# yifanlu0227/HEAL

Hardware: AMD Instinct MI355X
Metric: scenes/sec (5-agent OPV2V-H, PointPillars+PyramidFusion) (higher is better)
Workload: dtype f32

## Files before the change

heal_amd/_capi.py:

```python
import ctypes
import os
import re

HERE = os.path.dirname(os.path.abspath(__file__))
LIB_PATH = os.environ.get("HEAL_AMD_LIB") or os.path.join(HERE, "lib", "libheal_amd.so")
HEADER = os.path.join(os.path.dirname(HERE), "include", "heal_amd.h")
HEADER_EXPERIMENTAL = os.path.join(os.path.dirname(HERE), "include", "heal_amd_experimental.h")

_lib = None

c_void_p, c_int, c_float, c_size_t = ctypes.c_void_p, ctypes.c_int, ctypes.c_float, ctypes.c_size_t

_SIGNATURES = {
    "heal_abi_version": (c_int, []),
    "heal_last_error": (ctypes.c_char_p, []),
    "heal_fill_bytes": (c_int, [c_void_p, c_int, c_size_t, c_void_p]),
    "heal_next_launch_events": (c_int, [c_void_p, c_void_p]),
    "heal_voxelize_workspace": (c_size_t, [c_int, c_int, c_int, ctypes.c_longlong]),
    "heal_voxelize": (c_int, [c_void_p, c_int, c_void_p, c_void_p, c_int, c_int, c_int,
                              c_void_p, c_void_p, c_void_p, c_void_p, c_void_p, c_void_p, c_void_p, c_size_t, c_int, c_void_p]),
    "heal_voxelize_batch_workspace": (c_size_t, [c_int, c_int, c_int, c_int, ctypes.c_longlong]),
    "heal_voxelize_batch": (c_int, [c_void_p, c_void_p, c_int, c_void_p, c_void_p, c_int, c_int, c_void_p, c_void_p,
                                    c_void_p, c_void_p, c_void_p, c_size_t, c_int, c_void_p]),
    "heal_mask_points": (c_int, [c_void_p, c_int, c_void_p, c_int, c_void_p, c_void_p]),
    "heal_pfn_scatter_workspace": (c_size_t, [c_int] * 5),
    "heal_pfn_scatter": (c_int, [c_void_p, c_void_p, c_void_p, c_int, c_void_p, c_int,
                                 c_void_p, c_void_p, c_void_p, c_int,
                                 c_float, c_float, c_float, c_float, c_float, c_float,
                                 c_int, c_int, c_int, c_void_p, c_void_p, c_void_p, c_size_t, c_void_p]),
    "heal_pfn_pillars": (c_int, [c_void_p, c_void_p, c_void_p, c_int, c_void_p, c_int, c_void_p, c_void_p, c_void_p, c_int,
                                 c_float, c_float, c_float, c_float, c_float, c_float, c_int, c_int, c_int, c_void_p, c_void_p,
                                 c_void_p]),
    "heal_pillar_canvas": (c_int, [c_void_p, c_void_p, c_int, c_int, c_int, c_int, c_void_p, c_void_p]),
    "heal_pillar_stem_block": (c_int, [c_void_p, c_void_p, c_int, c_int, c_int, c_int] + [c_void_p] * 4 + [c_int] + [c_void_p] * 3),
    "heal_bev_pool_backward": (c_int, [c_void_p] * 5 + [c_int] * 6 + [c_void_p] * 6),
    "heal_warp_fuse": (c_int, [c_void_p, c_void_p, c_int, c_int, c_int, c_int, c_void_p, c_void_p, c_int, c_void_p,
                               c_void_p, c_void_p]),
    "heal_warp_fuse_levels": (c_int, [c_int, c_void_p, c_void_p, c_int, c_void_p, c_void_p, c_void_p, c_void_p, c_void_p, c_int,
                                      c_void_p, c_void_p, c_void_p]),
    "heal_warp_att_fuse_levels": (c_int, [c_int, c_void_p, c_int, c_void_p, c_void_p, c_void_p, c_void_p, c_void_p, c_void_p, c_int,
                                          c_int, c_void_p, c_void_p]),
    "heal_disco_fuse": (c_int, [c_void_p, c_int, c_int, c_int, c_int, c_void_p, c_void_p, c_int] + [c_void_p] * 11),
    "heal_warp_fuse_backward": (c_int, [c_void_p, c_void_p, c_int, c_int, c_int, c_int, c_void_p, c_void_p, c_int, c_void_p,
                                        c_void_p, c_void_p, c_void_p, c_void_p]),
    "heal_warp_agent": (c_int, [c_void_p, c_void_p, c_int, c_int, c_int, c_void_p, c_void_p, c_int, c_void_p,
                                c_void_p, c_void_p, c_void_p]),
    "heal_warp_agents_pm": (c_int, [c_void_p, c_int, c_int, c_int, c_int, c_void_p, c_void_p, c_int, c_void_p, c_void_p]),
    "heal_fuse_warped": (c_int, [c_void_p, c_void_p, c_int, c_int, c_int, c_int, c_void_p, c_void_p]),
    "heal_fuse_warped_rows": (c_int, [c_void_p, c_void_p, c_void_p, c_int, c_int, c_int, c_int, c_void_p, c_void_p]),
    "heal_decode_nms_workspace": (c_size_t, [c_int, c_int]),
    "heal_decode_nms": (c_int, [c_void_p, c_void_p, c_void_p, c_void_p, c_int, c_int, c_int, c_int,
                                c_float, c_float, c_float, c_int, c_void_p, c_void_p,
                                c_void_p, c_void_p, c_void_p, c_int, c_void_p, c_size_t, c_void_p]),
    "heal_decode_nms_agents_workspace": (c_size_t, [c_int, c_int]),
# ... 283 lines not shown
```

heal_amd/csrc/warp_fuse.hip:

```cpp
#include <stdlib.h>
#include "common.h"
#include "warp_taps.h"
#include "../../include/heal_amd.h"

namespace heal {

constexpr int WF_TW = 32, WF_TH = 8;

struct WarpParams {
    const double* mdev;
    double m[WF_MAXA][6];
    int crop[WF_MAXA][4];
    int n_agents, C, H, W;
    int grid_f64;
};

__device__ __forceinline__ void load_affine(const WarpParams& p, int a, double (&m)[6]) {
#pragma unroll
    for (int k = 0; k < 6; ++k) m[k] = p.mdev ? p.mdev[a * 6 + k] : p.m[a][k];
}

__device__ __forceinline__ float score_at(const float* __restrict__ occ, int idx, int W, const int* crop) {
    if (crop[1] > crop[0]) {
        const int h = idx / W, w = idx - h * W;
// ... 107 lines not shown
                    }
                }
            }
        }
#pragma unroll
        for (int u = 0; u < U; ++u)
            if (c + u < p.C) out[(size_t)(c + u) * HW + pix] = acc[u];
    }
}

constexpr int WL_T = 16;
constexpr int WL_BMAX = 32;
constexpr int WL_CC = 8;
constexpr int WL_MAXL = 4;

struct WfLevel {
    const float* feats;
    const float* occ;
    float* out;
    int C, H, W;
    int tiles_x, cgroups, cpb;
    int block0;
    int crop[WF_MAXA][4];
};
struct WfLevels {
    WfLevel lv[WL_MAXL];
    int n_levels, n_agents, grid_f64, dbg;
    const double* mdev;
    double m[WF_MAXA][6];
};

template <int NA>
__global__ __launch_bounds__(256) void k_warp_fuse_lds(const WfLevels P) {
    __shared__ float s_box_f[WL_CC * WL_BMAX * (WL_BMAX + 1)];
    __shared__ int s_box[WF_MAXA][4];
    int lvl = 0;
#pragma unroll
    for (int i = 1; i < WL_MAXL; ++i)
        if (i < P.n_levels && (int)blockIdx.x >= P.lv[i].block0) lvl = i;
    const WfLevel& L = P.lv[lvl];
    const int lb = blockIdx.x - L.block0;
    const int cg = lb % L.cgroups, tile = lb / L.cgroups;
    const int tx0 = (tile % L.tiles_x) * WL_T, ty0 = (tile / L.tiles_x) * WL_T;
    const int tid = threadIdx.x;
    const int w = tx0 + (tid & (WL_T - 1)), h = ty0 + (tid >> 4);
// ... 23 lines not shown
        for (int k = 0; k < 4; ++k) wt[a][k] = 0.f;
        if (live) {
            float gx, gy;
            double m[6];
#pragma unroll
            for (int k = 0; k < 6; ++k) m[k] = P.mdev ? P.mdev[a * 6 + k] : P.m[a][k];
            if (P.grid_f64) {
                const double xs = s_base_d[0][tid & (WL_T - 1)], ys = s_base_d[1][tid >> 4];
                gx = (float)((m[0] * xs + m[1] * ys) + m[2]);
                gy = (float)((m[3] * xs + m[4] * ys) + m[5]);
            } else {
                const float xs = s_base_f[0][tid & (WL_T - 1)], ys = s_base_f[1][tid >> 4];
                gx = (float)(((float)m[0] * xs + (float)m[1] * ys) + (float)m[2]);
                gy = (float)(((float)m[3] * xs + (float)m[4] * ys) + (float)m[5]);
            }
            const Taps t = make_taps(gx, gy, L.H, L.W);
            prob[a] = sample_score(L.occ + (size_t)a * HW, t, L.W, L.crop[a]);
            const float ix = ((gx + 1.f) * (float)L.W - 1.f) / 2.f, iy = ((gy + 1.f) * (float)L.H - 1.f) / 2.f;
            tx[a] = (int)fminf(fmaxf(floorf(ix), -2.f), (float)L.W);
            ty[a] = (int)fminf(fmaxf(floorf(iy), -2.f), (float)L.H);
            okb[a] = t.ok;
#pragma unroll
            for (int k = 0; k < 4; ++k) wt[a][k] = ((t.ok >> k) & 1u) ? t.w[k] : 0.f;
        }
    }
    agent_softmax(prob, NA);
#pragma unroll
    for (int a = 0; a < NA; ++a) {
#pragma unroll
        for (int k = 0; k < 4; ++k) wt[a][k] *= prob[a];
        const bool any = (wt[a][0] != 0.f) | (wt[a][1] != 0.f) | (wt[a][2] != 0.f) | (wt[a][3] != 0.f);
        if (!any) okb[a] = 0u;
        int x_lo = any ? ((okb[a] & 5u) ? tx[a] : tx[a] + 1) : (1 << 30), x_hi = any ? ((okb[a] & 10u) ? tx[a] + 1 : tx[a]) : -(1 << 30);
        int y_lo = any ? ((okb[a] & 3u) ? ty[a] : ty[a] + 1) : (1 << 30), y_hi = any ? ((okb[a] & 12u) ? ty[a] + 1 : ty[a]) : -(1 << 30);
#pragma unroll
// ... 8 lines not shown
    }
    __syncthreads();

    const int c_lo = cg * L.cpb, c_hi = (P.dbg & 1) ? c_lo : min(c_lo + L.cpb, L.C);
    const int pix = h * L.W + w;
    const int lx = tid & 31, ry = tid >> 5;
    for (int c0 = c_lo; c0 < c_hi; c0 += WL_CC) {
        float acc[WL_CC];
#pragma unroll
        for (int u = 0; u < WL_CC; ++u) acc[u] = 0.f;
        const int nc = min(WL_CC, c_hi - c0);
#pragma unroll
        for (int a = 0; a < NA; ++a) {
            const int bx0 = s_box[a][0], by0 = s_box[a][1], bw = s_box[a][2] - bx0 + 1, bh = s_box[a][3] - by0 + 1;
            if (bw <= 0 || bh <= 0) continue;
            const float* __restrict__ base = L.feats + ((size_t)a * L.C + c0) * HW;
            if (bw <= WL_BMAX && bh <= WL_BMAX) {
                const int pitch = bw | 1;
                float st[4][WL_CC];
                const int xs = min(lx, bw - 1);
#pragma unroll
                for (int j = 0; j < 4; ++j) {
                    const float* rowp = base + (size_t)(by0 + min(ry + 8 * j, bh - 1)) * L.W + bx0 + xs;
#pragma unroll
                    for (int u = 0; u < WL_CC; ++u) st[j][u] = (P.dbg & 2) ? 1.f : rowp[(size_t)min(u, nc - 1) * HW];
                }
#pragma unroll
                for (int j = 0; j < 4; ++j) {
                    const int y = ry + 8 * j;
                    if (lx < bw && y < bh) {
#pragma unroll
                        for (int u = 0; u < WL_CC; ++u)
                            if (u < nc) s_box_f[(u * bh + y) * pitch + lx] = st[j][u];
                    }
                }
                __syncthreads();
                if (okb[a] && !(P.dbg & 4)) {
                    const int o = (ty[a] - by0) * pitch + (tx[a] - bx0);
                    const int o0 = (okb[a] & 1u) ? o : 0, o1 = (okb[a] & 2u) ? o + 1 : 0;
                    const int o2 = (okb[a] & 4u) ? o + pitch : 0, o3 = (okb[a] & 8u) ? o + pitch + 1 : 0;
#pragma unroll
                    for (int u = 0; u < WL_CC; ++u) {
                        if (u < nc) {
                            const float* s = s_box_f + u * bh * pitch;
                            float v = s[o0] * wt[a][0];
                            v += s[o1] * wt[a][1];
                            v += s[o2] * wt[a][2];
                            v += s[o3] * wt[a][3];
                            acc[u] += v;
                        }
                    }
                }
                __syncthreads();
            } else if (okb[a]) {
                const int o = ty[a] * L.W + tx[a];
                const int o0 = (okb[a] & 1u) ? o : 0, o1 = (okb[a] & 2u) ? o + 1 : 0;
                const int o2 = (okb[a] & 4u) ? o + L.W : 0, o3 = (okb[a] & 8u) ? o + L.W + 1 : 0;
#pragma unroll
                for (int u = 0; u < WL_CC; ++u) {
                    if (u < nc) {
                        const float* src = base + (size_t)u * HW;
                        float v = src[o0] * wt[a][0];
                        v += src[o1] * wt[a][1];
                        v += src[o2] * wt[a][2];
                        v += src[o3] * wt[a][3];
                        acc[u] += v;
                    }
                }
            }
        }
        if (live) {
#pragma unroll
            for (int u = 0; u < WL_CC; ++u)
                if (u < nc) L.out[(size_t)(c0 + u) * HW + pix] = acc[u];
        }
    }
// ... 312 lines not shown
    int cch = (int)(((long long)channels * tiles + 1023) / 1024);
    cch = (cch + 3) / 4 * 4;
    if (cch < 4) cch = 4;
    if (cch > channels) cch = (channels + 3) / 4 * 4;
    dim3 grid(ceil_div(W, WF_TW), ceil_div(H, WF_TH), ceil_div(channels, cch));
    hipStream_t st = (hipStream_t)stream;
    switch (n_agents) {
#define HEAL_WF(N) case N: k_warp_fuse<N><<<grid, 256, 0, st>>>(feats, occ, p, cch, out); break;
        HEAL_WF(1) HEAL_WF(2) HEAL_WF(3) HEAL_WF(4) HEAL_WF(5) HEAL_WF(6) HEAL_WF(7) HEAL_WF(8)
#undef HEAL_WF
    }
    HEAL_LAUNCH_CHECK();
    return 0;
}

extern "C" int heal_warp_fuse_levels(int n_levels, const float* const* feats_host, const float* const* occ_host,
                                     int n_agents, const int32_t* channels_host, const int32_t* h_host, const int32_t* w_host,
                                     const double* affine_host, const double* affine_dev, int grid_f64,
                                     const int32_t* crop_host, float* const* out_host, void* stream) {
    HEAL_REQUIRE(n_levels >= 1 && n_levels <= WL_MAXL, "warp_fuse_levels: 1..%d levels per launch (got %d)", WL_MAXL, n_levels);
    HEAL_REQUIRE(n_agents >= 1 && n_agents <= WF_MAXA, "warp_fuse_levels: n_agents must be in [1,%d] (got %d)", WF_MAXA, n_agents);
    HEAL_REQUIRE(affine_host != nullptr || affine_dev != nullptr, "warp_fuse_levels: affine is NULL (host and device)");
    WfLevels P;
    P.n_levels = n_levels; P.n_agents = n_agents; P.grid_f64 = grid_f64; P.mdev = affine_dev;
    P.dbg = HEAL_DEBUG_ENV("HEAL_K5_DBG");
    for (int a = 0; a < WF_MAXA; ++a)
        for (int k = 0; k < 6; ++k) P.m[a][k] = (a < n_agents && affine_host) ? affine_host[a * 6 + k] : 0.0;
    long long blocks = 0;
    for (int l = 0; l < WL_MAXL; ++l) {
        WfLevel& L = P.lv[l];
        if (l >= n_levels) { L = P.lv[0]; L.block0 = 1 << 30; continue; }
        HEAL_REQUIRE(feats_host[l] && occ_host[l] && out_host[l] && channels_host[l] >= 1 && h_host[l] >= 1 && w_host[l] >= 1,
                     "warp_fuse_levels: bad level %d", l);
        L.feats = feats_host[l]; L.occ = occ_host[l]; L.out = out_host[l];
        L.C = channels_host[l]; L.H = h_host[l]; L.W = w_host[l];
        L.tiles_x = ceil_div(L.W, WL_T);
        const int tiles = L.tiles_x * ceil_div(L.H, WL_T);
        int target = 512;
        static const int env_blocks = [] { const char* e = getenv("HEAL_K5_BLOCKS"); return e ? atoi(e) : 0; }();
        if (env_blocks > 0) target = env_blocks;
        int cg = (int)((target + tiles - 1) / tiles);
        cg = cg < 1 ? 1 : cg;
        int cpb = ceil_div(ceil_div(L.C, cg), WL_CC) * WL_CC;
        L.cpb = cpb;
        L.cgroups = ceil_div(L.C, cpb);
        L.block0 = (int)blocks;
        blocks += (long long)tiles * L.cgroups;
        for (int a = 0; a < WF_MAXA; ++a)
            for (int k = 0; k < 4; ++k)
                L.crop[a][k] = (a < n_agents && crop_host) ? crop_host[((size_t)l * n_agents + a) * 4 + k] : 0;
    }
    HEAL_REQUIRE(blocks < (1ll << 30), "warp_fuse_levels: grid too large");
    hipStream_t st = (hipStream_t)stream;
    switch (n_agents) {
#define HEAL_WFL(N) case N: HEAL_LAUNCH_EV(k_warp_fuse_lds<N>, dim3((unsigned)blocks), dim3(256), 0, st, P); break;
        HEAL_WFL(1) HEAL_WFL(2) HEAL_WFL(3) HEAL_WFL(4) HEAL_WFL(5) HEAL_WFL(6) HEAL_WFL(7) HEAL_WFL(8)
#undef HEAL_WFL
    }
    HEAL_LAUNCH_CHECK();
    return 0;
}

extern "C" int heal_warp_att_fuse_levels(int n_levels, const float* const* feats_host, int n_agents, const int32_t* channels_host,
                                         const int32_t* h_host, const int32_t* w_host, const float* sqrt_dim_host,
                                         const double* affine_host, const double* affine_dev, int grid_f64, int mode,
                                         float* const* out_host, void* stream) {
    HEAL_REQUIRE(n_levels >= 1 && n_levels <= WL_MAXL, "warp_att_fuse_levels: 1..%d levels per launch (got %d)", WL_MAXL, n_levels);
    HEAL_REQUIRE(n_agents >= 1 && n_agents <= WF_MAXA, "warp_att_fuse_levels: n_agents must be in [1,%d] (got %d)", WF_MAXA, n_agents);
    HEAL_REQUIRE(mode == 0 || mode == 1, "warp_att_fuse_levels: mode must be 0 (attention) or 1 (max), got %d", mode);
    HEAL_REQUIRE(feats_host && out_host && channels_host && h_host && w_host, "warp_att_fuse_levels: null argument");
    HEAL_REQUIRE(affine_host != nullptr || affine_dev != nullptr, "warp_att_fuse_levels: affine is NULL (host and device)");
    WaLevels P;
    P.n_levels = n_levels; P.n_agents = n_agents; P.grid_f64 = grid_f64; P.mode = mode; P.mdev = affine_dev;
    for (int a = 0; a < WF_MAXA; ++a)
        for (int k = 0; k < 6; ++k) P.m[a][k] = (a < n_agents && affine_host) ? affine_host[a * 6 + k] : 0.0;
// ... 109 lines not shown
```

heal_amd/opencood/models/_heter_common.py:

```python
import importlib
from collections import OrderedDict

import torch
import torch.nn.functional as F

from heal_amd.derived import derived


def modality_names(args):
    return [x for x in args.keys() if x.startswith("m") and x[1:].isdigit()]


def find_encoder(core_method):
    lib = importlib.import_module("heal_amd.opencood.models.heter_encoders")
    target = core_method.replace("_", "").lower()
    for name, cls in lib.__dict__.items():
        if name.lower() == target:
            return cls
    raise KeyError(f"encoder '{core_method}' not found in heter_encoders")


def modality_stems(model, args, make_backbone):
    model.modality_name_list = modality_names(args)
    model.cav_range = args["lidar_range"]
# ... 10 lines not shown
        if setting["sensor_type"] == "camera":
            grid = setting["camera_mask_args"]["grid_conf"]
            setattr(model, f"crop_ratio_W_{m}", model.cav_range[3] / grid["xbound"][1])
            setattr(model, f"crop_ratio_H_{m}", model.cav_range[4] / grid["ybound"][1])
        yield m, setting


def crop_camera_feature(model, m, feature):
    if model.sensor_type_dict[m] != "camera":
        return feature
    H, W = (int(v) for v in feature.shape[-2:])
    th, tw = int(H * getattr(model, f"crop_ratio_H_{m}")), int(W * getattr(model, f"crop_ratio_W_{m}"))
    boxes = model.__dict__.setdefault("_heal_cam_boxes", {})
    if th > H and tw > W:
        boxes[m] = ((th - H) // 2, (th - H) // 2 + H, (tw - W) // 2, (tw - W) // 2 + W)
    else:
        boxes.pop(m, None)
    return center_crop(feature, th, tw)


def wants_depth_items(model, m):
    return model.sensor_type_dict[m] == "camera" and bool(getattr(model, f"depth_supervision_{m}"))


def anchor_heads(in_channels, args):
    import torch.nn as nn
    a = args["anchor_number"]
    return (nn.Conv2d(in_channels, a, kernel_size=1), nn.Conv2d(in_channels, 7 * a, kernel_size=1),
            nn.Conv2d(in_channels, args["dir_args"]["num_bins"] * a, kernel_size=1))


def center_crop(x, target_h, target_w):
    H, W = x.shape[-2:]
# ... 106 lines not shown
```

heal_amd/opencood/models/fuse_modules/pyramid_fuse.py:

```python
import torch
import torch.nn as nn

from heal_amd import derived, ops
from heal_amd.opencood.models.sub_modules.bev_blocks import (Bottleneck, ResNetBEVBackbone, ResNetModified)


def crop_window(H, W, ratio_h, ratio_w):
    crop_H = H / ratio_h - 4
    crop_W = W / ratio_w - 4
    return (int(H // 2 - crop_H // 2), int(H // 2 + crop_H // 2),
            int(W // 2 - crop_W // 2), int(W // 2 + crop_W // 2))


def weighted_fuse_autograd(x, occ, record_len, affine_matrix, crops=None):
    import torch.nn.functional as F
    score = torch.sigmoid(occ) + 1e-4
    if crops is not None:
        keep = torch.ones_like(score)
        for a, c in enumerate(crops):
            if c is not None:
                keep[a] = 0
                keep[a, :, c[0]:c[1], c[2]:c[3]] = 1
        score = score * keep
    out, start = [], 0
# ... 166 lines not shown
            return None
        boxes = [cam_boxes[agent_modality_list[k]] for k in cams]
        box = (min(b[0] for b in boxes), max(b[1] for b in boxes), min(b[2] for b in boxes), max(b[3] for b in boxes))
        H, W = int(spatial_features.shape[2]), int(spatial_features.shape[3])
        if H % 32 or W % 32 or not (0 <= box[0] < box[1] <= H and 0 <= box[2] < box[3] <= W):
            return None
        if derived.capturing() and not derived.ready(*self._zero_response_slot(spatial_features)):
            return None
        return (cams[0], cams[-1] + 1), box

    def multiscale(self, spatial_features, agent_modality_list=None, cam_boxes=None):
        cc = self._camcrop_args(spatial_features, agent_modality_list, cam_boxes)
        if cc is not None:
            return self.get_multiscale_feature_camcrop(spatial_features, *cc)
        return self.get_multiscale_feature(spatial_features)

    def forward_collab(self, spatial_features, record_len, affine_matrix, agent_modality_list=None,
                       cam_crop_info=None, grid_f64=True, cam_boxes=None):
        feature_list = self.multiscale(spatial_features, agent_modality_list, cam_boxes if len(record_len) == 1 else None)
        use_crop = bool(cam_crop_info) and not self.training
        fused_feature_list, occ_map_list = [], []
        import os
        if (len(record_len) == 1 and not torch.is_grad_enabled() and feature_list[0].is_cuda and 1 <= self.num_levels <= 4
                and int(record_len[0]) <= 8 and os.environ.get("HEAL_K5_LEVELS", "1") == "1"):
            n = int(record_len[0])
            crops_all = []
            for i in range(self.num_levels):
                occ_map_list.append(self.occupancy_head(i, feature_list[i]))
                crops = None
                if use_crop:
# ... 24 lines not shown
```

heal_amd/opencood/models/heter_pyramid_collab.py:

```python
from collections import Counter

import torch
import torch.nn as nn

from heal_amd.opencood.models._heter_common import (anchor_heads, crop_camera_feature, detection_heads, encode_modalities,
                                                     modality_stems, record_len_to_list, wants_depth_items)
from heal_amd.opencood.models.fuse_modules.pyramid_fuse import PyramidFusion
from heal_amd.opencood.models.sub_modules.bev_blocks import (AlignNet, DownsampleConv, NaiveCompressor,
                                                             ResNetBEVBackbone)
from heal_amd.opencood.utils.transformation_utils import normalize_pairwise_tfm, pairwise_to_host


class HeterPyramidCollab(nn.Module):
    def __init__(self, args):
        super().__init__()
        self.args = args
        self.cam_crop_info = {}
        for m, setting in modality_stems(self, args, lambda st: ResNetBEVBackbone(st["backbone_args"])):
            setattr(self, f"aligner_{m}", AlignNet(setting["aligner_args"]))
            if setting["sensor_type"] == "camera":
                grid = setting["camera_mask_args"]["grid_conf"]
                setattr(self, f"xdist_{m}", grid["xbound"][1] - grid["xbound"][0])
                setattr(self, f"ydist_{m}", grid["ybound"][1] - grid["ybound"][0])
                self.cam_crop_info[m] = {f"crop_ratio_W_{m}": getattr(self, f"crop_ratio_W_{m}"),
# ... 24 lines not shown
        return self.encode_modality_tail(m, getattr(self, f"encoder_{m}")(data_dict, m))

    def encode_modality_head(self, data_dict, m):
        enc = getattr(self, f"encoder_{m}")
        return enc.forward_head(data_dict, m) if hasattr(enc, "forward_head") else enc(data_dict, m)

    def encode_modality_tail(self, m, feature):
        feature = getattr(self, f"backbone_{m}")({"spatial_features": feature})["spatial_features_2d"]
        return crop_camera_feature(self, m, getattr(self, f"aligner_{m}")(feature))

    def heads(self, fused_feature):
        if self.shrink_flag:
            fused_feature = self.shrink_conv(fused_feature)
        return detection_heads(fused_feature, self.cls_head, self.reg_head, self.dir_head)

    def forward(self, data_dict):
        output_dict = {"pyramid": "collab"}
        agent_modality_list = data_dict["agent_modality_list"]
        pairwise, grid_f64 = pairwise_to_host(data_dict["pairwise_t_matrix"])
        affine_matrix = normalize_pairwise_tfm(pairwise, self.H, self.W, self.fake_voxel_size)
        record_len = record_len_to_list(data_dict["record_len"])
        counts = Counter(agent_modality_list)
        feats = encode_modalities(self, data_dict, counts, self.encode_modality)
        for m in feats:
            if wants_depth_items(self, m):
                output_dict[f"depth_items_{m}"] = getattr(self, f"encoder_{m}").depth_items
        if len(feats) == 1 and len(counts) == 1:
            heter_feature_2d = next(iter(feats.values()))
        else:
            cursor = {m: 0 for m in self.modality_name_list}
            parts = []
            for m in agent_modality_list:
                parts.append(feats[m][cursor[m]])
                cursor[m] += 1
            heter_feature_2d = torch.stack(parts)
        cam_boxes = None
        if self.compress:
            heter_feature_2d = self.compressor(heter_feature_2d)
        else:
            cam_boxes = {m: b for m, b in self.__dict__.get("_heal_cam_boxes", {}).items() if m in feats}
        fused, occ_outputs = self.pyramid_backbone.forward_collab(
# ... 6 lines not shown
```

heal_amd/ops.py:

```python
import ctypes
import os

import numpy as np
import torch

from . import _capi, derived
from .derived import derived as _derived

_WS = {}

TIMING = None
SP_TRACE = None
LAST_CALLS = None


def _remember(name, fn):
    if LAST_CALLS is not None:
        LAST_CALLS[name] = fn


def graph_period_ms(fn, reps=20, iters=10):
    global TIMING, LAST_CALLS
    saved = (TIMING, LAST_CALLS)
    TIMING, LAST_CALLS = None, None
# ... 507 lines not shown
    cp, carr = ctypes.c_void_p(0), None
    if crops is not None and any(c is not None for c in crops):
        carr = np.zeros((L, n, 4), dtype=np.int32)
        for l, c in enumerate(crops):
            if c is not None:
                carr[l] = np.asarray([ci if ci is not None else (0, 0, 0, 0) for ci in c], dtype=np.int32).reshape(n, 4)
        cp = carr.ctypes.data_as(ctypes.c_void_p)
    fp = _host_array([f.data_ptr() for f in feats_list], ctypes.c_void_p)
    op = _host_array([o.data_ptr() for o in occ_list], ctypes.c_void_p)
    yp = _host_array([y.data_ptr() for y in outs], ctypes.c_void_p)
    with _Timed("warp_fuse_levels", 0.0, nbytes, kernel_events=True):
        _capi.call("heal_warp_fuse_levels", L, fp, op, n, _host_array([int(f.shape[1]) for f in feats_list], ctypes.c_int32),
                   _host_array([int(f.shape[2]) for f in feats_list], ctypes.c_int32),
                   _host_array([int(f.shape[3]) for f in feats_list], ctypes.c_int32), ap, adev, int(bool(grid_f64)), cp, yp,
                   _stream())
    return outs


WARP_ATT_MAX_AGENTS, WARP_ATT_MAX_LEVELS = 8, 4


def warp_att_fuse_levels(feats_list, affine_rows, grid_f64=True, mode="att", sqrt_dims=None):
    if mode not in ("att", "max"):
        raise _capi.HealAmdError(f"warp_att_fuse_levels: mode must be 'att' or 'max', got {mode!r}")
    L = len(feats_list)
    if not 1 <= L <= WARP_ATT_MAX_LEVELS:
        raise _capi.HealAmdError(f"warp_att_fuse_levels: 1..{WARP_ATT_MAX_LEVELS} levels per launch (got {L})")
    feats_list = [_need(f, torch.float32, "feats") for f in feats_list]
    if any(f.dim() != 4 for f in feats_list):
        raise _capi.HealAmdError("warp_att_fuse_levels: every level must be [n, C, H, W]")
# ... 1741 lines not shown
```

heal_amd/pipeline.py:

```python
import numpy as np
import torch

from heal_amd import _capi, synth
from heal_amd.opencood.data_utils.post_processor.voxel_postprocessor import VoxelPostprocessor
from heal_amd.opencood.tools.train_utils import create_model


def fill_deterministic(module, seed=0):
    g = torch.Generator().manual_seed(seed)
    with torch.no_grad():
        for name, t in module.state_dict().items():
            if not t.dtype.is_floating_point:
                continue
            leaf = name.rsplit(".", 1)[-1]
            if leaf == "running_var":
                t.copy_(0.7 + 0.6 * torch.rand(t.shape, generator=g))
            elif leaf == "running_mean":
                t.copy_(0.1 * torch.randn(t.shape, generator=g))
            elif t.dim() == 1 and leaf == "weight":
                t.copy_(1.0 + 0.1 * torch.randn(t.shape, generator=g))
            elif leaf in ("bias", "gamma"):
                t.copy_(0.05 * torch.randn(t.shape, generator=g))
            elif t.dim() >= 2:
                fan_in = int(np.prod(t.shape[1:]))
# ... 157 lines not shown
        self.device = torch.device(device)
        self.model = fill_deterministic(create_model(hypes), seed).to(self.device).eval()
        self.post = VoxelPostprocessor(hypes["postprocess"], train=False)
        self.anchor_box = torch.from_numpy(self.post.generate_anchor_box()).to(self.device)
        self.tfm = torch.eye(4)

    @torch.no_grad()
    def calibrate_cls_bias(self, scene, target_candidates=600):
        return calibrate_heads(self.model, scene.model_input(),
                               self.hypes["postprocess"]["target_args"]["score_threshold"], target_candidates)

    @torch.no_grad()
    def forward(self, scene):
        return self.model(scene.model_input())

    @torch.no_grad()
    def step(self, scene):
        out = self.model(scene.model_input())
        batch = {"ego": {"transformation_matrix": self.tfm, "anchor_box": self.anchor_box}}
        return self.post.post_process(batch, {"ego": out})

    def _device_step(self, inputs):
        from heal_amd import ops
        dir_args = self.post.params.get("dir_args", {"dir_offset": 0.7853, "num_bins": 2})
        anchors = self.post._anchors_f32(self.anchor_box, self.device)
        out = self.model(inputs.model_input())
        return ops.decode_nms(out["cls_preds"], out["reg_preds"], out.get("dir_preds"), anchors,
                              self.post.params["target_args"]["score_threshold"], dir_args["dir_offset"],
                              dir_args["num_bins"], self.post.params["nms_thresh"],
                              np.eye(4, dtype=np.float32), self.post.params["gt_range"], sync=False)

    @torch.no_grad()
    def capture_slot(self, scene, warmup=3, slack=1.25):
        from heal_amd import ops
        static = StaticInputs(scene, slack)

        def body():
            return self._device_step(static)

        cur = torch.cuda.current_stream(self.device)
        if cur == torch.cuda.default_stream(self.device):
# ... 157 lines not shown
```

include/heal_amd.h:

```cpp
#ifndef HEAL_AMD_H
#define HEAL_AMD_H

#include <stddef.h>
#include <stdint.h>

#ifdef __cplusplus
extern "C" {
#endif

#define HEAL_AMD_ABI_VERSION 12

int heal_abi_version(void);
const char* heal_last_error(void);

int heal_fill_bytes(void* dst, int byte, size_t bytes, void* stream);
int heal_next_launch_events(void* start_event, void* stop_event);

size_t heal_voxelize_workspace(int n_points, int max_points, int max_voxels, long long agents_x_cells);
int heal_voxelize(const float* points, int n_points,
                  const float* range_host, const float* voxel_size_host,
                  int max_points, int max_voxels, int batch_idx,
                  float* voxels, int32_t* coords, int32_t* num_points, int32_t* n_voxels,
                  const int32_t* row_offset, int32_t* row_offset_next,
                  void* ws, size_t ws_bytes, int tables_clean, void* stream);
// ... 22 lines not shown
                     float z_offset, int n_agents, int ny, int nx, float* pillar_feat, int32_t* cell_map, void* stream);
int heal_pillar_canvas(const int32_t* cell_map, const float* pillar_feat, int n_agents, int channels, int ny, int nx,
                       float* canvas, void* stream);
int heal_pillar_stem_block(const float* pillar_feat, const int32_t* cell_map, int n_agents, int channels, int ny, int nx,
                           const float* w_main, const float* b_main, const float* w_down, const float* b_down,
                           int weight_layout, float* out_main, float* out_identity, void* stream);

int heal_warp_fuse(const float* feats, const float* occ, int n_agents, int channels, int H, int W,
                   const double* affine_host, const double* affine_dev, int grid_f64,
                   const int32_t* crop_host, float* out, void* stream);

int heal_warp_fuse_levels(int n_levels, const float* const* feats_host, const float* const* occ_host, int n_agents,
                          const int32_t* channels_host, const int32_t* h_host, const int32_t* w_host,
                          const double* affine_host, const double* affine_dev, int grid_f64, const int32_t* crop_host,
                          float* const* out_host, void* stream);

int heal_warp_att_fuse_levels(int n_levels, const float* const* feats_host, int n_agents, const int32_t* channels_host,
                              const int32_t* h_host, const int32_t* w_host, const float* sqrt_dim_host,
                              const double* affine_host, const double* affine_dev, int grid_f64, int mode,
                              float* const* out_host, void* stream);

int heal_disco_fuse(const float* feats, int n_agents, int channels, int H, int W, const double* affine_host,
                    const double* affine_dev, int grid_f64, const float* e0, const float* w1n_frag, const float* w2_frag,
                    const float* b2, const float* w3, const float* b3, const float* w4, const float* b4, float* out,
                    float* scores, void* stream);

int heal_warp_fuse_backward(const float* feats, const float* occ, int n_agents, int channels, int H, int W,
                            const double* affine_host, const double* affine_dev, int grid_f64, const int32_t* crop_host,
                            const float* grad_out, float* grad_feats, float* grad_occ, void* stream);

// ... 262 lines not shown
```

Before: 162.1.

## Warp-fuse camera features from unpadded boxes instead of zero-padded full maps

Adds a per-agent source descriptor (pointer, strides, valid box) to the multi-level warp-fuse kernel so it can sample directly from strided sub-views. A lean inference path skips center-crop padding of camera features and runs the pyramid collab step on these unpadded views. This removes the pad copies and the zero reads over padded regions, at the cost of extra bounds checks per tap and a more complex host planning path.

```diff
diff --git a/heal_amd/_capi.py b/heal_amd/_capi.py
--- a/heal_amd/_capi.py
+++ b/heal_amd/_capi.py
@@ -38,6 +38,8 @@
                                c_void_p, c_void_p]),
     "heal_warp_fuse_levels": (c_int, [c_int, c_void_p, c_void_p, c_int, c_void_p, c_void_p, c_void_p, c_void_p, c_void_p, c_int,
                                       c_void_p, c_void_p, c_void_p]),
+    "heal_warp_fuse_levels_src": (c_int, [c_int, c_void_p, c_int, c_void_p, c_void_p, c_void_p, c_void_p, c_void_p, c_int,
+                                          c_void_p, c_void_p, c_void_p]),
     "heal_warp_att_fuse_levels": (c_int, [c_int, c_void_p, c_int, c_void_p, c_void_p, c_void_p, c_void_p, c_void_p, c_void_p, c_int,
                                           c_int, c_void_p, c_void_p]),
     "heal_disco_fuse": (c_int, [c_void_p, c_int, c_int, c_int, c_int, c_void_p, c_void_p, c_int] + [c_void_p] * 11),
diff --git a/heal_amd/csrc/warp_fuse.hip b/heal_amd/csrc/warp_fuse.hip
--- a/heal_amd/csrc/warp_fuse.hip
+++ b/heal_amd/csrc/warp_fuse.hip
@@ -145,14 +145,19 @@
 constexpr int WL_CC = 8;
 constexpr int WL_MAXL = 4;
 
+struct WfSource {
+    const float* feat;
+    const float* occ;
+    int row, plane, orow;
+    int box[4];
+    int keep[4];
+};
 struct WfLevel {
-    const float* feats;
-    const float* occ;
+    WfSource src[WF_MAXA];
     float* out;
     int C, H, W;
     int tiles_x, cgroups, cpb;
     int block0;
-    int crop[WF_MAXA][4];
 };
 struct WfLevels {
     WfLevel lv[WL_MAXL];
@@ -160,6 +165,20 @@
     const double* mdev;
     double m[WF_MAXA][6];
 };
+
+__device__ __forceinline__ float score_src(const WfSource& S, int y, int x) {
+    if (y < S.keep[0] || y >= S.keep[1] || x < S.keep[2] || x >= S.keep[3]) return 0.f;
+    return 1.f / (1.f + expf(-S.occ[(size_t)(y - S.box[0]) * S.orow + (x - S.box[2])])) + 1e-4f;
+}
+
+__device__ __forceinline__ float sample_score_src(const WfSource& S, const Taps& t, int ty, int tx) {
+    float acc = 0.f;
+    if (t.ok & 1u) acc = score_src(S, ty, tx) * t.w[0];
+    if (t.ok & 2u) acc += score_src(S, ty, tx + 1) * t.w[1];
+    if (t.ok & 4u) acc += score_src(S, ty + 1, tx) * t.w[2];
+    if (t.ok & 8u) acc += score_src(S, ty + 1, tx + 1) * t.w[3];
+    return acc;
+}
 
 template <int NA>
 __global__ __launch_bounds__(256) void k_warp_fuse_lds(const WfLevels P) {
@@ -213,11 +232,15 @@
                 gx = (float)(((float)m[0] * xs + (float)m[1] * ys) + (float)m[2]);
                 gy = (float)(((float)m[3] * xs + (float)m[4] * ys) + (float)m[5]);
             }
-            const Taps t = make_taps(gx, gy, L.H, L.W);
-            prob[a] = sample_score(L.occ + (size_t)a * HW, t, L.W, L.crop[a]);
+            Taps t = make_taps(gx, gy, L.H, L.W);
             const float ix = ((gx + 1.f) * (float)L.W - 1.f) / 2.f, iy = ((gy + 1.f) * (float)L.H - 1.f) / 2.f;
             tx[a] = (int)fminf(fmaxf(floorf(ix), -2.f), (float)L.W);
             ty[a] = (int)fminf(fmaxf(floorf(iy), -2.f), (float)L.H);
+            const WfSource& S = L.src[a];
+            const unsigned in_y0 = ty[a] >= S.box[0] && ty[a] < S.box[1], in_y1 = ty[a] + 1 >= S.box[0] && ty[a] + 1 < S.box[1];
+            const unsigned in_x0 = tx[a] >= S.box[2] && tx[a] < S.box[3], in_x1 = tx[a] + 1 >= S.box[2] && tx[a] + 1 < S.box[3];
+            t.ok &= (in_y0 & in_x0) | ((in_y0 & in_x1) << 1) | ((in_y1 & in_x0) << 2) | ((in_y1 & in_x1) << 3);
+            prob[a] = sample_score_src(S, t, ty[a], tx[a]);
             okb[a] = t.ok;
 #pragma unroll
             for (int k = 0; k < 4; ++k) wt[a][k] = ((t.ok >> k) & 1u) ? t.w[k] : 0.f;
@@ -256,16 +279,19 @@
         for (int a = 0; a < NA; ++a) {
             const int bx0 = s_box[a][0], by0 = s_box[a][1], bw = s_box[a][2] - bx0 + 1, bh = s_box[a][3] - by0 + 1;
             if (bw <= 0 || bh <= 0) continue;
-            const float* __restrict__ base = L.feats + ((size_t)a * L.C + c0) * HW;
+            const WfSource& S = L.src[a];
+            const int row = S.row;
+            const size_t plane = (size_t)S.plane;
+            const float* __restrict__ base = S.feat + (size_t)c0 * plane + (size_t)(by0 - S.box[0]) * row + (bx0 - S.box[2]);
             if (bw <= WL_BMAX && bh <= WL_BMAX) {
                 const int pitch = bw | 1;
                 float st[4][WL_CC];
                 const int xs = min(lx, bw - 1);
 #pragma unroll
                 for (int j = 0; j < 4; ++j) {
-                    const float* rowp = base + (size_t)(by0 + min(ry + 8 * j, bh - 1)) * L.W + bx0 + xs;
-#pragma unroll
-                    for (int u = 0; u < WL_CC; ++u) st[j][u] = (P.dbg & 2) ? 1.f : rowp[(size_t)min(u, nc - 1) * HW];
+                    const float* rowp = base + (size_t)min(ry + 8 * j, bh - 1) * row + xs;
+#pragma unroll
+                    for (int u = 0; u < WL_CC; ++u) st[j][u] = (P.dbg & 2) ? 1.f : rowp[(size_t)min(u, nc - 1) * plane];
                 }
 #pragma unroll
                 for (int j = 0; j < 4; ++j) {
@@ -295,13 +321,13 @@
                 }
                 __syncthreads();
             } else if (okb[a]) {
-                const int o = ty[a] * L.W + tx[a];
+                const int o = (ty[a] - by0) * row + (tx[a] - bx0);
                 const int o0 = (okb[a] & 1u) ? o : 0, o1 = (okb[a] & 2u) ? o + 1 : 0;
-                const int o2 = (okb[a] & 4u) ? o + L.W : 0, o3 = (okb[a] & 8u) ? o + L.W + 1 : 0;
+                const int o2 = (okb[a] & 4u) ? o + row : 0, o3 = (okb[a] & 8u) ? o + row + 1 : 0;
 #pragma unroll
                 for (int u = 0; u < WL_CC; ++u) {
                     if (u < nc) {
-                        const float* src = base + (size_t)u * HW;
+                        const float* src = base + (size_t)u * plane;
                         float v = src[o0] * wt[a][0];
                         v += src[o1] * wt[a][1];
                         v += src[o2] * wt[a][2];
@@ -644,13 +670,10 @@
     return 0;
 }
 
-extern "C" int heal_warp_fuse_levels(int n_levels, const float* const* feats_host, const float* const* occ_host,
-                                     int n_agents, const int32_t* channels_host, const int32_t* h_host, const int32_t* w_host,
-                                     const double* affine_host, const double* affine_dev, int grid_f64,
-                                     const int32_t* crop_host, float* const* out_host, void* stream) {
-    HEAL_REQUIRE(n_levels >= 1 && n_levels <= WL_MAXL, "warp_fuse_levels: 1..%d levels per launch (got %d)", WL_MAXL, n_levels);
-    HEAL_REQUIRE(n_agents >= 1 && n_agents <= WF_MAXA, "warp_fuse_levels: n_agents must be in [1,%d] (got %d)", WF_MAXA, n_agents);
-    HEAL_REQUIRE(affine_host != nullptr || affine_dev != nullptr, "warp_fuse_levels: affine is NULL (host and device)");
+static int launch_warp_fuse_levels(const char* who, int n_levels, const heal_k5_source* src_host, int n_agents,
+                                   const int32_t* channels_host, const int32_t* h_host, const int32_t* w_host,
+                                   const double* affine_host, const double* affine_dev, int grid_f64, const int32_t* crop_host,
+                                   float* const* out_host, void* stream) {
     WfLevels P;
     P.n_levels = n_levels; P.n_agents = n_agents; P.grid_f64 = grid_f64; P.mdev = affine_dev;
     P.dbg = HEAL_DEBUG_ENV("HEAL_K5_DBG");
@@ -660,9 +683,8 @@
     for (int l = 0; l < WL_MAXL; ++l) {
         WfLevel& L = P.lv[l];
         if (l >= n_levels) { L = P.lv[0]; L.block0 = 1 << 30; continue; }
-        HEAL_REQUIRE(feats_host[l] && occ_host[l] && out_host[l] && channels_host[l] >= 1 && h_host[l] >= 1 && w_host[l] >= 1,
-                     "warp_fuse_levels: bad level %d", l);
-        L.feats = feats_host[l]; L.occ = occ_host[l]; L.out = out_host[l];
+        HEAL_REQUIRE(out_host[l] && channels_host[l] >= 1 && h_host[l] >= 1 && w_host[l] >= 1, "%s: bad level %d", who, l);
+        L.out = out_host[l];
         L.C = channels_host[l]; L.H = h_host[l]; L.W = w_host[l];
         L.tiles_x = ceil_div(L.W, WL_T);
         const int tiles = L.tiles_x * ceil_div(L.H, WL_T);
@@ -676,11 +698,30 @@
         L.cgroups = ceil_div(L.C, cpb);
         L.block0 = (int)blocks;
         blocks += (long long)tiles * L.cgroups;
-        for (int a = 0; a < WF_MAXA; ++a)
-            for (int k = 0; k < 4; ++k)
-                L.crop[a][k] = (a < n_agents && crop_host) ? crop_host[((size_t)l * n_agents + a) * 4 + k] : 0;
-    }
-    HEAL_REQUIRE(blocks < (1ll << 30), "warp_fuse_levels: grid too large");
+        for (int a = 0; a < WF_MAXA; ++a) {
+            WfSource& S = L.src[a];
+            if (a >= n_agents) { S = L.src[0]; continue; }
+            const heal_k5_source& h = src_host[(size_t)l * n_agents + a];
+            const int* b = h.box;
+            HEAL_REQUIRE(h.feat && h.occ, "%s: level %d agent %d: null source", who, l, a);
+            HEAL_REQUIRE(0 <= b[0] && b[0] < b[1] && b[1] <= L.H && 0 <= b[2] && b[2] < b[3] && b[3] <= L.W,
+                         "%s: level %d agent %d: box (%d,%d,%d,%d) is empty or leaves the %d x %d map", who, l, a, b[0], b[1], b[2],
+                         b[3], L.H, L.W);
+            const long long bh = b[1] - b[0], bw = b[3] - b[2];
+            HEAL_REQUIRE(h.feat_row >= bw && h.occ_row >= bw && h.feat_plane >= (bh - 1) * h.feat_row + bw &&
+                             h.feat_plane < (1ll << 31) && (long long)L.C * h.feat_plane < (1ll << 40),
+                         "%s: level %d agent %d: strides (row %lld, plane %lld, occ row %lld) do not hold a %lld x %lld box", who, l, a,
+                         (long long)h.feat_row, (long long)h.feat_plane, (long long)h.occ_row, bh, bw);
+            S.feat = h.feat; S.occ = h.occ;
+            S.row = (int)h.feat_row; S.plane = (int)h.feat_plane; S.orow = (int)h.occ_row;
+            const int32_t* c = crop_host ? crop_host + ((size_t)l * n_agents + a) * 4 : nullptr;
+            const bool window = c && c[1] > c[0];
+            for (int k = 0; k < 4; ++k) S.box[k] = b[k];
+            S.keep[0] = window ? (c[0] > b[0] ? c[0] : b[0]) : b[0]; S.keep[1] = window ? (c[1] < b[1] ? c[1] : b[1]) : b[1];
+            S.keep[2] = window ? (c[2] > b[2] ? c[2] : b[2]) : b[2]; S.keep[3] = window ? (c[3] < b[3] ? c[3] : b[3]) : b[3];
+        }
+    }
+    HEAL_REQUIRE(blocks < (1ll << 30), "%s: grid too large", who);
     hipStream_t st = (hipStream_t)stream;
     switch (n_agents) {
 #define HEAL_WFL(N) case N: HEAL_LAUNCH_EV(k_warp_fuse_lds<N>, dim3((unsigned)blocks), dim3(256), 0, st, P); break;
@@ -689,6 +730,66 @@
     }
     HEAL_LAUNCH_CHECK();
     return 0;
+}
+
+extern "C" int heal_warp_fuse_levels(int n_levels, const float* const* feats_host, const float* const* occ_host,
+                                     int n_agents, const int32_t* channels_host, const int32_t* h_host, const int32_t* w_host,
+                                     const double* affine_host, const double* affine_dev, int grid_f64,
+                                     const int32_t* crop_host, float* const* out_host, void* stream) {
+    HEAL_REQUIRE(n_levels >= 1 && n_levels <= WL_MAXL, "warp_fuse_levels: 1..%d levels per launch (got %d)", WL_MAXL, n_levels);
+    HEAL_REQUIRE(n_agents >= 1 && n_agents <= WF_MAXA, "warp_fuse_levels: n_agents must be in [1,%d] (got %d)", WF_MAXA, n_agents);
+    HEAL_REQUIRE(affine_host != nullptr || affine_dev != nullptr, "warp_fuse_levels: affine is NULL (host and device)");
+    heal_k5_source src[WL_MAXL * WF_MAXA];
+    for (int l = 0; l < n_levels; ++l) {
+        HEAL_REQUIRE(feats_host[l] && occ_host[l] && out_host[l] && channels_host[l] >= 1 && h_host[l] >= 1 && w_host[l] >= 1,
+                     "warp_fuse_levels: bad level %d", l);
+        const long long HW = (long long)h_host[l] * w_host[l];
+        for (int a = 0; a < n_agents; ++a) {
+            heal_k5_source& h = src[l * n_agents + a];
+            h.feat = feats_host[l] + (size_t)a * channels_host[l] * HW;
+            h.occ = occ_host[l] + (size_t)a * HW;
+            h.feat_row = w_host[l]; h.feat_plane = HW; h.occ_row = w_host[l];
+            h.box[0] = 0; h.box[1] = h_host[l]; h.box[2] = 0; h.box[3] = w_host[l];
+        }
+    }
+    return launch_warp_fuse_levels("warp_fuse_levels", n_levels, src, n_agents, channels_host, h_host, w_host, affine_host, affine_dev,
+                                   grid_f64, crop_host, out_host, stream);
+}
+
+extern "C" int heal_warp_fuse_levels_src(int n_levels, const heal_k5_source* src_host, int n_agents, const int32_t* channels_host,
+                                         const int32_t* h_host, const int32_t* w_host, const double* affine_host,
+                                         const double* affine_dev, int grid_f64, const int32_t* crop_host, float* const* out_host,
+                                         void* stream) {
+    HEAL_REQUIRE(n_levels >= 1 && n_levels <= WL_MAXL, "warp_fuse_levels_src: 1..%d levels per launch (got %d)", WL_MAXL, n_levels);
+    HEAL_REQUIRE(n_agents >= 1 && n_agents <= WF_MAXA, "warp_fuse_levels_src: n_agents must be in [1,%d] (got %d)", WF_MAXA, n_agents);
+    HEAL_REQUIRE(affine_host != nullptr || affine_dev != nullptr, "warp_fuse_levels_src: affine is NULL (host and device)");
+    HEAL_REQUIRE(src_host && channels_host && h_host && w_host && out_host, "warp_fuse_levels_src: null argument");
+    for (int l = 0; l < n_levels; ++l) {
+        const int H = h_host[l], W = w_host[l];
+        for (int a = 0; a < n_agents; ++a) {
+            const heal_k5_source& h = src_host[(size_t)l * n_agents + a];
+            const int* b = h.box;
+            const int32_t* c = crop_host ? crop_host + ((size_t)l * n_agents + a) * 4 : nullptr;
+            if (c && c[1] > c[0]) {
+                const int y0 = c[0] - 1 > 0 ? c[0] - 1 : 0, y1 = c[1] + 1 < H ? c[1] + 1 : H;
+                const int x0 = c[2] - 1 > 0 ? c[2] - 1 : 0, x1 = c[3] + 1 < W ? c[3] + 1 : W;
+                HEAL_REQUIRE(b[0] <= y0 && y1 <= b[1] && b[2] <= x0 && x1 <= b[3],
+                             "warp_fuse_levels_src: level %d agent %d: crop window (%d,%d,%d,%d) +- 1 is not inside its box (%d,%d,%d,%d)",
+                             l, a, c[0], c[1], c[2], c[3], b[0], b[1], b[2], b[3]);
+            } else {
+                HEAL_REQUIRE(b[0] == 0 && b[1] == H && b[2] == 0 && b[3] == W,
+                             "warp_fuse_levels_src: level %d agent %d has no crop window: its box must be the full %d x %d map (got "
+                             "(%d,%d,%d,%d))", l, a, H, W, b[0], b[1], b[2], b[3]);
+            }
+            HEAL_REQUIRE(h.feat_row % 4 == 0 && h.feat_plane % 4 == 0 && h.occ_row % 4 == 0 &&
+                             (((uintptr_t)h.feat >> 2) - (uintptr_t)b[2]) % 4 == 0 && ((uintptr_t)h.feat & 3) == 0 &&
+                             (((uintptr_t)h.occ >> 2) - (uintptr_t)b[2]) % 4 == 0 && ((uintptr_t)h.occ & 3) == 0,
+                         "warp_fuse_levels_src: level %d agent %d: misaligned box (strides must be multiples of 4 floats and column 0 "
+                         "of the map rows 16-byte aligned: pointer - 4 x0 bytes)", l, a);
+        }
+    }
+    return launch_warp_fuse_levels("warp_fuse_levels_src", n_levels, src_host, n_agents, channels_host, h_host, w_host, affine_host,
+                                   affine_dev, grid_f64, crop_host, out_host, stream);
 }
 
 extern "C" int heal_warp_att_fuse_levels(int n_levels, const float* const* feats_host, int n_agents, const int32_t* channels_host,
diff --git a/heal_amd/opencood/models/_heter_common.py b/heal_amd/opencood/models/_heter_common.py
--- a/heal_amd/opencood/models/_heter_common.py
+++ b/heal_amd/opencood/models/_heter_common.py
@@ -48,9 +48,15 @@
     boxes = model.__dict__.setdefault("_heal_cam_boxes", {})
     if th > H and tw > W:
         boxes[m] = ((th - H) // 2, (th - H) // 2 + H, (tw - W) // 2, (tw - W) // 2 + W)
+        if model.__dict__.get("_heal_lean_walk"):
+            model.__dict__.setdefault("_heal_cam_unpadded", {})[m] = (th, tw)
+            return feature
     else:
         boxes.pop(m, None)
     return center_crop(feature, th, tw)
+
+
+LEAN_WALK_KEY = "heal_lean_walk"
 
 
 def wants_depth_items(model, m):
diff --git a/heal_amd/opencood/models/fuse_modules/pyramid_fuse.py b/heal_amd/opencood/models/fuse_modules/pyramid_fuse.py
--- a/heal_amd/opencood/models/fuse_modules/pyramid_fuse.py
+++ b/heal_amd/opencood/models/fuse_modules/pyramid_fuse.py
@@ -204,6 +204,120 @@
         if cc is not None:
             return self.get_multiscale_feature_camcrop(spatial_features, *cc)
         return self.get_multiscale_feature(spatial_features)
+
+    def _zero_response_crop(self, like, level, crop):
+        tag, sources, extra = self._zero_response_slot(like)
+        return "pyramid_zero_response_crop", sources, extra + (int(level), tuple(int(v) for v in crop))
+
+    @staticmethod
+    def _cam_window(H, W, mod, cam_crop_info):
+        return crop_window(H, W, cam_crop_info[mod][f"crop_ratio_H_{mod}"], cam_crop_info[mod][f"crop_ratio_W_{mod}"])
+
+    def lean_plan(self, like, record_len, agent_modality_list, cam_boxes, cam_crop_info):
+        import os
+        if (len(record_len) != 1 or not 1 <= self.num_levels <= 4 or int(record_len[0]) > 8 or self.training
+                or os.environ.get("HEAL_K5_LEVELS", "1") != "1" or os.environ.get("HEAL_PYRAMID_LEAN", "1") != "1"):
+            return None
+        cc = self._camcrop_args(like, agent_modality_list, cam_boxes)
+        if cc is None:
+            return None
+        (c0, c1), box = cc
+        n = len(agent_modality_list)
+        other = (0, c0) if c0 > 0 else (c1, n)
+        if not cam_crop_info or any(agent_modality_list[k] not in cam_crop_info for k in range(c0, c1)):
+            return None
+        if len({agent_modality_list[k] for k in range(*other)}) > 1:
+            return None
+        plan = self._camcrop_plan(like, (c0, c1), box)
+        if plan[0] is None:
+            return None
+        H, W = int(like.shape[2]), int(like.shape[3])
+        gbox = plan[0][1]
+        for k in range(c0, c1):
+            wy0, wy1, wx0, wx1 = self._cam_window(H, W, agent_modality_list[k], cam_crop_info)
+            if not (gbox[0] <= max(0, wy0 - 1) and min(H, wy1 + 1) <= gbox[1] and gbox[2] <= max(0, wx0 - 1) and min(W, wx1 + 1) <= gbox[3]):
+                return None
+        if self.layernum_ > 1 and plan[1] is not None:
+            slot = self._zero_response_crop(like, 0, plan[1][0])
+            if derived.capturing() and not derived.ready(slot[0], slot[1], slot[2]):
+                return None
+        return (c0, c1), other, plan
+
+    def forward_collab_lean(self, lidar, cam_maps, like, lean, affine_matrix, agent_modality_list, cam_crop_info, cam_boxes,
+                            grid_f64=True):
+        (c0, c1), other, plan = lean
+        n, nc, nl = len(agent_modality_list), c1 - c0, other[1] - other[0]
+        bg = self._zero_response(like)
+        dt, dev = like.dtype, like.device
+        (cy0, cy1, cx0, cx1), gbox, pbox = plan[0]
+        layer = self.resnet.layer0
+        xc = torch.zeros((nc, int(like.shape[1]), cy1 - cy0, cx1 - cx0), dtype=dt, device=dev)
+        for j, m in enumerate(cam_maps):
+            b = cam_boxes[agent_modality_list[c0 + j]]
+            xc[j, :, b[0] - cy0:b[1] - cy0, b[2] - cx0:b[3] - cx0] = m
+        yc = layer(xc)
+        full, xl = None, None
+        if self.layernum_ > 1 and plan[1] is None:
+            full = torch.empty((n,) + tuple(bg[0].shape[1:]), dtype=dt, device=dev)
+            full[c0:c1] = bg[0]
+            full[c0:c1, :, gbox[0]:gbox[1], gbox[2]:gbox[3]] = yc[:, :, pbox[0]:pbox[1], pbox[2]:pbox[3]]
+        if nl:
+            xl = lidar
+            for j, blk in enumerate(layer):
+                xl = blk(xl, out=full[other[0]:other[1]]) if (full is not None and j == len(layer) - 1) else blk(xl)
+        sources, shapes = [], []
+        occ_c = self.occupancy_head(0, yc)
+        occ_l = self.occupancy_head(0, xl) if nl else None
+        level = [None] * n
+        for j in range(nl):
+            level[other[0] + j] = (xl[j], occ_l[j, 0], (0, 0))
+        for j in range(nc):
+            level[c0 + j] = (yc[j, :, pbox[0]:pbox[1], pbox[2]:pbox[3]], occ_c[j, 0, pbox[0]:pbox[1], pbox[2]:pbox[3]],
+                             (gbox[0], gbox[2]))
+        sources.append(level)
+        shapes.append(tuple(int(v) for v in bg[0].shape[2:]))
+        for i in range(1, self.layernum_):
+            layer = getattr(self.resnet, f"layer{i}")
+            if plan[i] is None:
+                full = self.resnet.run_stage(layer, full)
+            else:
+                (cy0, cy1, cx0, cx1), g2, p2 = plan[i]
+                nxt = torch.empty((n,) + tuple(bg[i].shape[1:]), dtype=dt, device=dev)
+                if nl:
+                    xa = full[other[0]:other[1]] if full is not None else xl
+                    for j, blk in enumerate(layer):
+                        xa = blk(xa, out=nxt[other[0]:other[1]]) if j == len(layer) - 1 else blk(xa)
+                if full is not None:
+                    xin = full[c0:c1, :, cy0:cy1, cx0:cx1].contiguous()
+                else:
+                    crop = (cy0, cy1, cx0, cx1)
+                    tag, src, extra = self._zero_response_crop(like, i - 1, crop)
+                    bgc = derived.derived(tag, src, lambda: bg[i - 1][:, :, cy0:cy1, cx0:cx1].contiguous(), extra)
+                    xin = bgc.repeat(nc, 1, 1, 1)
+                    iy0, iy1, ix0, ix1 = max(gbox[0], cy0), min(gbox[1], cy1), max(gbox[2], cx0), min(gbox[3], cx1)
+                    xin[:, :, iy0 - cy0:iy1 - cy0, ix0 - cx0:ix1 - cx0] = yc[:, :, pbox[0] + iy0 - gbox[0]:pbox[0] + iy1 - gbox[0],
+                                                                             pbox[2] + ix0 - gbox[2]:pbox[2] + ix1 - gbox[2]]
+                yc = layer(xin)
+                nxt[c0:c1] = bg[i]
+                nxt[c0:c1, :, g2[0]:g2[1], g2[2]:g2[3]] = yc[:, :, p2[0]:p2[1], p2[2]:p2[3]]
+                gbox, pbox, full = g2, p2, nxt
+            occ = self.occupancy_head(i, full)
+            H, W = int(full.shape[2]), int(full.shape[3])
+            level = []
+            for k in range(n):
+                y0, y1, x0, x1 = 0, H, 0, W
+                if c0 <= k < c1:
+                    wy0, wy1, wx0, wx1 = self._cam_window(H, W, agent_modality_list[k], cam_crop_info)
+                    y0, y1 = max(0, wy0 - 1), min(H, wy1 + 1)
+                    x0, x1 = max(0, wx0 - 1) // 4 * 4, min(W, -(-(wx1 + 1) // 4) * 4)
+                level.append((full[k, :, y0:y1, x0:x1], occ[k, 0, y0:y1, x0:x1], (y0, x0)))
+            sources.append(level)
+            shapes.append((H, W))
+        crops_all = []
+        for (H, W) in shapes:
+            crops_all.append([self._cam_window(H, W, mod, cam_crop_info) if mod in cam_crop_info else None for mod in agent_modality_list])
+        fused = ops.warp_fuse_levels_src(sources, shapes, affine_matrix[0][0, :n], grid_f64, crops_all)
+        return self.decode_multiscale_feature([f.unsqueeze(0) for f in fused])
 
     def forward_collab(self, spatial_features, record_len, affine_matrix, agent_modality_list=None,
                        cam_crop_info=None, grid_f64=True, cam_boxes=None):
diff --git a/heal_amd/opencood/models/heter_pyramid_collab.py b/heal_amd/opencood/models/heter_pyramid_collab.py
--- a/heal_amd/opencood/models/heter_pyramid_collab.py
+++ b/heal_amd/opencood/models/heter_pyramid_collab.py
@@ -3,8 +3,8 @@
 import torch
 import torch.nn as nn
 
-from heal_amd.opencood.models._heter_common import (anchor_heads, crop_camera_feature, detection_heads, encode_modalities,
-                                                     modality_stems, record_len_to_list, wants_depth_items)
+from heal_amd.opencood.models._heter_common import (LEAN_WALK_KEY, anchor_heads, center_crop, crop_camera_feature, detection_heads,
+                                                     encode_modalities, modality_stems, record_len_to_list, wants_depth_items)
 from heal_amd.opencood.models.fuse_modules.pyramid_fuse import PyramidFusion
 from heal_amd.opencood.models.sub_modules.bev_blocks import (AlignNet, DownsampleConv, NaiveCompressor,
                                                              ResNetBEVBackbone)
@@ -62,6 +62,32 @@
             fused_feature = self.shrink_conv(fused_feature)
         return detection_heads(fused_feature, self.cls_head, self.reg_head, self.dir_head)
 
+    def _lean_inputs(self, feats, unpadded, agent_modality_list, record_len):
+        cam_boxes = {m: b for m, b in self.__dict__.get("_heal_cam_boxes", {}).items() if m in feats}
+        if set(cam_boxes) != set(unpadded) or len({v for v in unpadded.values()}) != 1:
+            return None
+        others = [m for m in feats if m not in unpadded]
+        if len(others) > 1:
+            return None
+        H, W = next(iter(unpadded.values()))
+        cam0 = feats[next(iter(unpadded))]
+        lidar = feats[others[0]] if others else None
+        if lidar is not None and (tuple(lidar.shape[1:]) != (int(cam0.shape[1]), H, W) or lidar.dtype != cam0.dtype):
+            return None
+        if any(tuple(feats[m].shape[2:]) != (cam_boxes[m][1] - cam_boxes[m][0], cam_boxes[m][3] - cam_boxes[m][2]) for m in unpadded):
+            return None
+        like = lidar if lidar is not None else cam0.new_empty((0, int(cam0.shape[1]), H, W))
+        plan = self.pyramid_backbone.lean_plan(like, record_len, agent_modality_list, cam_boxes, self.cam_crop_info)
+        if plan is None:
+            return None
+        cursor = {m: 0 for m in unpadded}
+        cam_maps = []
+        for m in agent_modality_list:
+            if m in unpadded:
+                cam_maps.append(feats[m][cursor[m]])
+                cursor[m] += 1
+        return lidar, cam_maps, like, plan, cam_boxes
+
     def forward(self, data_dict):
         output_dict = {"pyramid": "collab"}
         agent_modality_list = data_dict["agent_modality_list"]
@@ -69,10 +95,27 @@
         affine_matrix = normalize_pairwise_tfm(pairwise, self.H, self.W, self.fake_voxel_size)
         record_len = record_len_to_list(data_dict["record_len"])
         counts = Counter(agent_modality_list)
-        feats = encode_modalities(self, data_dict, counts, self.encode_modality)
+        self.__dict__["_heal_lean_walk"] = bool(data_dict.get(LEAN_WALK_KEY)) and not self.compress and not torch.is_grad_enabled()
+        self.__dict__["_heal_cam_unpadded"] = {}
+        try:
+            feats = encode_modalities(self, data_dict, counts, self.encode_modality)
+        finally:
+            self.__dict__["_heal_lean_walk"] = False
+        unpadded = self.__dict__.pop("_heal_cam_unpadded")
         for m in feats:
             if wants_depth_items(self, m):
                 output_dict[f"depth_items_{m}"] = getattr(self, f"encoder_{m}").depth_items
+        if unpadded:
+            lean = self._lean_inputs(feats, unpadded, agent_modality_list, record_len)
+            if lean is not None:
+                lidar, cam_maps, like, plan, cam_boxes = lean
+                fused = self.pyramid_backbone.forward_collab_lean(lidar, cam_maps, like, plan, affine_matrix, agent_modality_list,
+                                                                  self.cam_crop_info, cam_boxes, grid_f64)
+                cls_preds, reg_preds, dir_preds = self.heads(fused)
+                output_dict.update({"cls_preds": cls_preds, "reg_preds": reg_preds, "dir_preds": dir_preds})
+                return output_dict
+            for m, (th, tw) in unpadded.items():
+                feats[m] = center_crop(feats[m], th, tw)
         if len(feats) == 1 and len(counts) == 1:
             heter_feature_2d = next(iter(feats.values()))
         else:
diff --git a/heal_amd/ops.py b/heal_amd/ops.py
--- a/heal_amd/ops.py
+++ b/heal_amd/ops.py
@@ -545,6 +545,59 @@
                    _host_array([int(f.shape[2]) for f in feats_list], ctypes.c_int32),
                    _host_array([int(f.shape[3]) for f in feats_list], ctypes.c_int32), ap, adev, int(bool(grid_f64)), cp, yp,
                    _stream())
+    return outs
+
+
+class K5Source(ctypes.Structure):
+    _fields_ = [("feat", ctypes.c_void_p), ("occ", ctypes.c_void_p), ("feat_row", ctypes.c_int64), ("feat_plane", ctypes.c_int64),
+                ("occ_row", ctypes.c_int64), ("box", ctypes.c_int32 * 4)]
+
+
+def warp_fuse_levels_src(sources, shapes, affine_rows, grid_f64=True, crops=None, outs=None):
+    L = len(sources)
+    n = len(sources[0])
+    desc = (K5Source * (L * n))()
+    given, outs = outs, []
+    chans, keep, nbytes = [], [], 0.0
+    for l, (level, (H, W)) in enumerate(zip(sources, shapes)):
+        if len(level) != n:
+            raise _capi.HealAmdError("warp_fuse_levels_src: every level needs one source per agent")
+        C = int(level[0][0].shape[0])
+        for a, (f, o, (y0, x0)) in enumerate(level):
+            for t, name in ((f, "feat"), (o, "occ")):
+                if not isinstance(t, torch.Tensor) or not t.is_cuda or t.dtype != torch.float32:
+                    raise _capi.HealAmdError(f"warp_fuse_levels_src: {name} must be a float32 CUDA/HIP tensor")
+            if (f.dim() != 3 or o.dim() != 2 or int(f.shape[0]) != C or tuple(f.shape[1:]) != tuple(o.shape)
+                    or (f.shape[2] > 1 and f.stride(2) != 1) or (o.shape[1] > 1 and o.stride(1) != 1)):
+                raise _capi.HealAmdError("warp_fuse_levels_src: feat [C, bh, bw] and occ [bh, bw] views with unit stride along x")
+            bh, bw = int(o.shape[0]), int(o.shape[1])
+            d = desc[l * n + a]
+            d.feat, d.occ = f.data_ptr(), o.data_ptr()
+            d.feat_row, d.feat_plane, d.occ_row = int(f.stride(1)), int(f.stride(0)), int(o.stride(0))
+            d.box[:] = [int(y0), int(y0) + bh, int(x0), int(x0) + bw]
+            keep += [f, o]
+            nbytes += 4.0 * bh * bw * (C + 1)
+        dev = level[0][0].device
+        if given is not None:
+            y = _need(given[l], torch.float32, "out")
+            if y is not given[l] or tuple(y.shape) != (C, int(H), int(W)):
+                raise _capi.HealAmdError("warp_fuse_levels_src: outs[l] must be a contiguous [C_l, H_l, W_l] tensor")
+        outs.append(given[l] if given is not None else torch.empty((C, int(H), int(W)), dtype=torch.float32, device=dev))
+        chans.append(C)
+        nbytes += 4.0 * C * H * W
+    a, ap, adev = _affine_args(affine_rows, n)
+    cp, carr = ctypes.c_void_p(0), None
+    if crops is not None and any(c is not None for c in crops):
+        carr = np.zeros((L, n, 4), dtype=np.int32)
+        for l, c in enumerate(crops):
+            if c is not None:
+                carr[l] = np.asarray([ci if ci is not None else (0, 0, 0, 0) for ci in c], dtype=np.int32).reshape(n, 4)
+        cp = carr.ctypes.data_as(ctypes.c_void_p)
+    yp = _host_array([y.data_ptr() for y in outs], ctypes.c_void_p)
+    with _Timed("warp_fuse_levels", 0.0, nbytes, kernel_events=True):
+        _capi.call("heal_warp_fuse_levels_src", L, ctypes.cast(desc, ctypes.c_void_p), n, _host_array(chans, ctypes.c_int32),
+                   _host_array([int(s[0]) for s in shapes], ctypes.c_int32), _host_array([int(s[1]) for s in shapes], ctypes.c_int32),
+                   ap, adev, int(bool(grid_f64)), cp, yp, _stream())
     return outs
 
 
diff --git a/heal_amd/pipeline.py b/heal_amd/pipeline.py
--- a/heal_amd/pipeline.py
+++ b/heal_amd/pipeline.py
@@ -195,9 +195,16 @@
     def forward(self, scene):
         return self.model(scene.model_input())
 
+    @staticmethod
+    def _lean_input(inputs):
+        from heal_amd.opencood.models._heter_common import LEAN_WALK_KEY
+        d = inputs.model_input()
+        d[LEAN_WALK_KEY] = True
+        return d
+
     @torch.no_grad()
     def step(self, scene):
-        out = self.model(scene.model_input())
+        out = self.model(self._lean_input(scene))
         batch = {"ego": {"transformation_matrix": self.tfm, "anchor_box": self.anchor_box}}
         return self.post.post_process(batch, {"ego": out})
 
@@ -205,7 +212,7 @@
         from heal_amd import ops
         dir_args = self.post.params.get("dir_args", {"dir_offset": 0.7853, "num_bins": 2})
         anchors = self.post._anchors_f32(self.anchor_box, self.device)
-        out = self.model(inputs.model_input())
+        out = self.model(self._lean_input(inputs))
         return ops.decode_nms(out["cls_preds"], out["reg_preds"], out.get("dir_preds"), anchors,
                               self.post.params["target_args"]["score_threshold"], dir_args["dir_offset"],
                               dir_args["num_bins"], self.post.params["nms_thresh"],
diff --git a/include/heal_amd.h b/include/heal_amd.h
--- a/include/heal_amd.h
+++ b/include/heal_amd.h
@@ -60,6 +60,16 @@
                           const int32_t* channels_host, const int32_t* h_host, const int32_t* w_host,
                           const double* affine_host, const double* affine_dev, int grid_f64, const int32_t* crop_host,
                           float* const* out_host, void* stream);
+
+typedef struct heal_k5_source {
+    const float* feat;
+    const float* occ;
+    int64_t feat_row, feat_plane, occ_row;
+    int32_t box[4];
+} heal_k5_source;
+int heal_warp_fuse_levels_src(int n_levels, const heal_k5_source* src_host, int n_agents, const int32_t* channels_host,
+                              const int32_t* h_host, const int32_t* w_host, const double* affine_host, const double* affine_dev,
+                              int grid_f64, const int32_t* crop_host, float* const* out_host, void* stream);
 
 int heal_warp_att_fuse_levels(int n_levels, const float* const* feats_host, int n_agents, const int32_t* channels_host,
                               const int32_t* h_host, const int32_t* w_host, const float* sqrt_dim_host,
```

Result: faster. 163.8, median of 6 (+1.1%).
